# rosielab/emojivoice

Measured on AMD Instinct MI355X. Metric: audio_seconds_per_second, higher is better.
Workload: dtype f32 (deep layers: operand = two block-scaled fp16 pieces, product = 3 fp16 products on the fp16 MFMA, f32 accumulate); 1 GPU; config2: batch 64 x 516-frame (5.99 s) utterances per GPU, 10 Euler steps + HiFi-GAN V1, 22.05 kHz; global_batch=64, frames=516, ode_steps=10, parallelism=dp1, collective=none, batch_pipeline=cfm(i+1) || hifigan(i) on two streams, 2 pipeline(s) in flight

## Files before the change

emojivoice_amd/_lib.py:

```python
from __future__ import annotations

import ctypes as C
import os
import subprocess
from typing import Dict, Optional

import numpy as np
import torch

_HERE = os.path.dirname(os.path.abspath(__file__))
LIB_PATH = os.environ.get("EV_LIB_PATH") or os.path.join(_HERE, "lib", "libemojivoice_hip.so")
CSRC = os.path.join(_HERE, "csrc")
SOURCES = [os.path.join(CSRC, n) for n in ("ev_engine.hip", "ev_kernels.h", "ev_analysis_kernels.h", "ev_analysis.h")] \
    + [os.path.join(os.path.dirname(_HERE), "include", "emojivoice.h")]

EXPORTS = [
    "ev_abi_version", "ev_create", "ev_destroy", "ev_last_error", "ev_load_estimator", "ev_load_vocoder", "ev_load_vocoder_cfg", "ev_load_text_encoder", "ev_text_encoder",
    "ev_text_encoder_status", "ev_stft_magnitude", "ev_denoise", "ev_align", "ev_dbg_conv_bench",
    "ev_workspace_bytes", "ev_cfm_decode", "ev_estimator", "ev_hifigan", "ev_profile_enable", "ev_profile_read", "ev_profile_read_split", "ev_dbg_last_cfg", "ev_set_arithmetic", "ev_get_arithmetic",
    "ev_op_conv1d", "ev_op_groupnorm_mish", "ev_op_groupnorm_mish2", "ev_op_conv_groupnorm", "ev_op_layernorm", "ev_op_split_pieces", "ev_op_attention", "ev_op_ln_mlp", "ev_set_mrf_streams_max",
    "ev_cfm_decode2", "ev_reserve", "ev_alloc_count", "ev_dbg_sk_stats", "ev_op_attn_out", "ev_dbg_set_amax", "ev_dbg_set_attn_h16", "ev_dbg_set_chain", "ev_dbg_sk_taken",
    "ev_load_mel_basis", "ev_mel_spectrogram",
    "ev_maximum_path", "ev_log_prior", "ev_mas_align",
    "ev_estimator_rows", "ev_cfm_loss",
    "ev_load_resampler", "ev_resample", "ev_mel_stats",
    "ev_trim_bounds", "ev_trim_apply",
    "ev_pitch_yin", "ev_dtw",
    "ev_loudness",
    "ev_pyin_observe", "ev_pyin_decode",
    "ev_op_attention2", "ev_op_attn_out2",
    "ev_load_stoi", "ev_stoi",
    "ev_load_stft_dist", "ev_stft_dist",
    "ev_load_voice_quality", "ev_voice_quality",
    "ev_load_formants", "ev_formants",
    "ev_perturbation",
    "ev_load_harmonics", "ev_harmonics",
    "ev_functionals",
]


class EvLibraryError(RuntimeError):
    pass


class ev_tensor_index(C.Structure):
    _fields_ = [("name", C.c_char_p), ("offset", C.c_uint64), ("ndim", C.c_int32), ("shape", C.c_int64 * 4)]


class ev_model_dims(C.Structure):
    _fields_ = [("n_feats", C.c_int32), ("spk_emb_dim", C.c_int32), ("channels", C.c_int32), ("heads", C.c_int32),
                ("head_dim", C.c_int32)]


class ev_vocoder_config(C.Structure):
    _fields_ = [("resblock", C.c_int32), ("num_levels", C.c_int32), ("upsample_rates", C.c_int32 * 4), ("upsample_kernel_sizes", C.c_int32 * 4),
                ("resblock_kernel_sizes", C.c_int32 * 3), ("resblock_dilations", (C.c_int32 * 3) * 3)]


def vocoder_config(h) -> ev_vocoder_config:
    c = ev_vocoder_config()
# ... 94 lines not shown
    lib.ev_stoi.argtypes = [vp, vp, vp, vp, i32, i32, C.c_double, C.c_double, vp, vp, vp, vp, vp, vp]
    lib.ev_load_stft_dist.argtypes = [vp, vp, vp, i32, i32, i32]
    lib.ev_stft_dist.argtypes = [vp, vp, vp, vp, i32, i32, C.c_double, vp, vp, vp, vp]
    lib.ev_load_voice_quality.argtypes = [vp, vp, vp, i32, i32, i32, vp, vp, i32, i32, i32, vp, C.c_double]
    lib.ev_voice_quality.argtypes = [vp, vp, vp, i32, i32, C.c_double, vp, vp, vp, vp]
    lib.ev_load_formants.argtypes = [vp, vp, i32, i32, i32, C.c_double, C.c_double, C.c_double, i32]
    lib.ev_formants.argtypes = [vp, vp, vp, i32, i32, C.c_double, vp, vp, vp, vp]
    lib.ev_perturbation.argtypes = [vp, vp, vp, i32, i32, i32, vp, i32, i32, C.c_double, C.c_double, C.c_double, vp, vp, vp, vp]
    lib.ev_load_harmonics.argtypes = [vp, vp, vp, i32, i32, i32, C.c_double, i32, C.c_double, C.c_double, C.c_double]
    lib.ev_harmonics.argtypes = [vp, vp, vp, i32, i32, vp, vp, vp, i32, C.c_double, vp, vp, vp, vp]
    lib.ev_functionals.argtypes = [vp, vp, vp, vp, i32, i32, i32, vp, i32, vp, vp, vp]
    lib.ev_maximum_path.argtypes = [vp, vp, vp, vp, i32, i32, i32, vp, vp, vp]
    lib.ev_log_prior.argtypes = [vp, vp, vp, i32, i32, i32, vp, vp]
    lib.ev_mas_align.argtypes = [vp, vp, vp, vp, vp, i32, i32, i32, vp, vp, vp, vp, vp]
    lib.ev_profile_enable.argtypes = [vp, i32]
    lib.ev_profile_read.argtypes = [vp, C.POINTER(C.c_double), C.POINTER(C.c_double), C.POINTER(C.c_int64), i32]
    lib.ev_profile_read_split.argtypes = [vp, C.POINTER(C.c_double), C.POINTER(C.c_double), C.POINTER(C.c_int64)]
    lib.ev_dbg_last_cfg.argtypes = [vp]
    lib.ev_set_arithmetic.argtypes = [vp, i32]
    lib.ev_get_arithmetic.argtypes = [vp]
    lib.ev_dbg_set_amax.argtypes = [vp, i32]
    lib.ev_dbg_set_attn_h16.argtypes = [vp, i32]
    lib.ev_dbg_set_chain.argtypes = [vp, i32]
    lib.ev_dbg_sk_taken.argtypes = [vp]
    lib.ev_dbg_sk_taken.restype = C.c_int64
    lib.ev_op_conv1d.argtypes = [vp, vp, vp, vp, i32, i32, i32, i32, i32, i32, i32, i32, i32, f32, vp, vp]
    lib.ev_op_groupnorm_mish.argtypes = [vp, vp, vp, vp, vp, i32, i32, i32, i32, vp, vp]
    lib.ev_op_groupnorm_mish2.argtypes = [vp, vp, vp, vp, vp, i32, i32, i32, i32, i32, vp, i32, vp, vp, vp]
    lib.ev_op_conv_groupnorm.argtypes = [vp, vp, vp, vp, i32, i32, i32, vp, vp, vp, i32, vp, vp, vp, vp, vp, C.POINTER(C.c_int), vp]
    lib.ev_op_layernorm.argtypes = [vp, vp, vp, vp, i32, i32, vp, vp]
    lib.ev_op_split_pieces.argtypes = [vp, vp, i32, vp, vp]
    lib.ev_op_attention.argtypes = [vp, vp, vp, i32, i32, i32, vp, vp]
    lib.ev_op_attn_out.argtypes = [vp, vp, vp, i32, i32, vp, vp, vp, vp]
    lib.ev_op_attention2.argtypes = [vp, vp, vp, i32, i32, i32, i32, i32, i32, vp, C.POINTER(C.c_int), vp]
    lib.ev_op_attn_out2.argtypes = [vp, vp, vp, i32, i32, i32, i32, vp, vp, f32, f32, f32, vp, C.POINTER(C.c_int), vp]
    lib.ev_op_ln_mlp.argtypes = [vp, vp, vp, vp, vp, vp, vp, vp, vp, vp, vp, i32, i32, i32, vp, vp]
    for n in EXPORTS:
        getattr(lib, n)
    _lib = lib
    return lib


def _stream_ptr() -> int:
    return int(torch.cuda.current_stream().cuda_stream)


# ... 621 lines not shown
        return int(self.lib.ev_workspace_bytes(self.h, B, Tp, Tv))

    def profile_enable(self, on: bool):
        self._check(self.lib.ev_profile_enable(self.h, int(on)), "ev_profile_enable")

    def op_split_pieces(self, x):
        x = self._f32(x).reshape(-1)
        out = torch.empty((3, x.numel()), dtype=torch.float32, device=x.device)
        self._check(self.lib.ev_op_split_pieces(self.h, x.data_ptr(), x.numel(), out.data_ptr(), _stream_ptr()), "ev_op_split_pieces")
        return out

    def set_arithmetic(self, bf16_products: int):
        self._check(self.lib.ev_set_arithmetic(self.h, int(bf16_products)), "ev_set_arithmetic")

    def set_amax(self, on: bool) -> None:
        self._check(self.lib.ev_dbg_set_amax(self.h, int(bool(on))), "ev_dbg_set_amax")

    def set_attn_h16(self, on: bool) -> None:
        self._check(self.lib.ev_dbg_set_attn_h16(self.h, int(bool(on))), "ev_dbg_set_attn_h16")

    def set_chain(self, on: bool) -> None:
        self._check(self.lib.ev_dbg_set_chain(self.h, int(bool(on))), "ev_dbg_set_chain")

    def arithmetic(self) -> int:
        return int(self.lib.ev_get_arithmetic(self.h))

    def last_cfg(self) -> int:
        return int(self.lib.ev_dbg_last_cfg(self.h))

    def profile_read_split(self):
        ms, fl, n = C.c_double(), C.c_double(), C.c_int64()
        self._check(self.lib.ev_profile_read_split(self.h, C.byref(ms), C.byref(fl), C.byref(n)), "ev_profile_read_split")
        return ms.value, fl.value, n.value

    def profile_read(self, reset: bool = True):
        ms, fl, n = C.c_double(), C.c_double(), C.c_int64()
        self._check(self.lib.ev_profile_read(self.h, C.byref(ms), C.byref(fl), C.byref(n), int(reset)), "ev_profile_read")
        return ms.value, fl.value, n.value

    def op_conv1d(self, x, w, bias, dilation=1, transposed=False, stride=1, padding=0, pre_lrelu_slope=-1.0):
        x = self._f32(x)
        B, Cin, T = x.shape
        w = np.ascontiguousarray(w.detach().cpu().float().numpy())
        if transposed:
            Cout, K = w.shape[1], w.shape[2]
            Tout = T * stride
# ... 139 lines not shown
```

emojivoice_amd/csrc/ev_engine.hip:

```cpp
#include "ev_kernels.h"
#include "../../include/emojivoice.h"

#include <math.h>
#include <stdlib.h>
#include <stdarg.h>
#include <stdio.h>
#include <string.h>

#include <algorithm>
#include <atomic>
#include <mutex>
#include <numeric>
#include <string>
#include <unordered_map>
#include <vector>

namespace {

struct HostTensor {
    const float* p = nullptr;
    int ndim = 0;
    int64_t shape[4] = {0, 0, 0, 0};
    int64_t numel() const { int64_t n = 1; for (int i = 0; i < ndim; ++i) n *= shape[i]; return n; }
};
typedef std::unordered_map<std::string, HostTensor> TensorMap;

struct Geom { int nrows, S, P, T; };

struct ConvLayer {
    float* W = nullptr;
    unsigned short* Wh = nullptr; float wh_scale = 1.f;
    unsigned short* Wx = nullptr;
    unsigned short* Wq = nullptr;
    float* bias = nullptr;
    int2* taplist[3] = {nullptr, nullptr, nullptr};
    int* nact[3] = {nullptr, nullptr, nullptr};
    bool sparse_taps = false;
    bool tile128_exact = true;
    int kstack_mt = 0, kstack_tap = 0;
    int ntaps = 0, off[EV_MAX_TAPS] = {0};
    int halo_lo = 0, halo_hi = 0;
    bool wide = false;
    int Cin = 0, Cout = 0, Mpad = 0, Kpad = 0;
    double macs_per_row = 0;
};

struct Epi {
    int act = ACT_NONE; float act_slope = 0.f; const float* act_a = nullptr; const float* act_b = nullptr;
    int mask1 = 0; float scale = 1.f; const float* R = nullptr; int ldr = 0; int accum = 0; int div3 = 0;
    int act2_lrelu = 0; float act2_slope = 0.f; int mask2 = 0; const float* rowmask = nullptr; int mmul = 1;
    float* Y2 = nullptr; int ldy2 = 0;
    float pro_slope = -1.f;
    int dbg = 0; int force_cfg = -1; int stagger = -1; unsigned long long* stamps = nullptr;
    float* gn_part = nullptr;
    int isplit_log2 = 31, isstride = 0;
    unsigned* ymax = nullptr; int ymax_mul = 1; const unsigned* rmax = nullptr; const unsigned* yold = nullptr; const unsigned* xmax = nullptr; int xmax_n = 0;
    int osplit_log2 = 31, osstride = 0;
};

struct ResnetW { ConvLayer c1r, c2; float *g1, *b1, *g2, *b2; };
struct TransW {
    ConvLayer qkv, out, ff1, ff2; float *ln1g, *ln1b, *ln3g, *ln3b, *alpha, *binv;
    float qkv_scale[3] = {0.f, 0.f, 0.f};
};

struct EstimatorW {
    bool loaded = false;
    int in_ch = 0;
    ConvLayer t1, t2, tmlp;
    ResnetW rn[6];
    ConvLayer rn0_c1r_x, rn0_c1r_ms;
    TransW tr[6];
    ConvLayer down0, down1, up0, up1, fin_conv, fin_proj;
    float *fin_g, *fin_b;
};

struct VocoderW {
    bool loaded = false;
    int rb = 1;
    int nl = 4;
// ... 42 lines not shown
    StoiW stoi;
    StftDistW stftd;
    VoiceQW voiceq;
    FormantW fmt;
    HarmW harm;
    struct Scratch { char* p = nullptr; size_t bytes = 0; hipStream_t last = nullptr; bool last_valid = false; };
    Scratch dn_ws, enc_ws, mas_ws;
    Scratch dtw_ws;
    Scratch stat_ws;
    Scratch trim_ws;
    Scratch loud_ws;
    Scratch stoi_ws;
    Scratch stftd_ws;
    float* zeros = nullptr;
    int max_steps = 64;
    int* bad_ids_host = nullptr; int* bad_ids_dev = nullptr;
    char* ws = nullptr; size_t ws_bytes = 0; size_t ws_used = 0; size_t ws_bytes_last = 0;
    int ws_B = -1, ws_Tp = -1, ws_Tv = -1;
    bool prof = false;
    bool fuse_pairs = true;
    bool fuse_attn = true;
    bool attn_h16 = true;
    bool use_chain = true;
    bool fuse_mlp = true;
    int gn_stats_tiles = 0;
    int fuse_mlp_min_tiles = 96;
    std::vector<hipEvent_t> ev_pool; size_t ev_used = 0;
    hipStream_t ws_stream = nullptr; bool ws_stream_valid = false;
    float* temb_host[2] = {nullptr, nullptr}; size_t temb_cap[2] = {0, 0}; hipEvent_t temb_ev[2] = {nullptr, nullptr}; int temb_slot = 0;
    float* cap_pool = nullptr; size_t cap_stride = 0; int cap_used = 0; int cap_nt[8] = {0};
    struct TprojEntry { int nt; float* d; };
    std::vector<TprojEntry> tproj_cache;
    bool captured = false; int cap_B = 0, cap_Tp = 0;
    int64_t n_allocs = 0;
    double prof_flops = 0; int64_t prof_launches = 0;
    struct ProfRec { int kind, Cin, Cout, ntaps, nrows, cfg, lean; double flops; bool split = false; };
    std::vector<ProfRec> prof_recs;
    hipStream_t stream = nullptr;
    hipStream_t mrf_stream[2] = {nullptr, nullptr};
    hipEvent_t mrf_ev[4] = {nullptr, nullptr, nullptr, nullptr};
    int ncu = 0;
    unsigned* sk_ctrl = nullptr;
    unsigned sk_seq = 0;
    float* sk_part = nullptr;
    int split_terms = 16;
    bool use_amax = true;
// ... 247 lines not shown
            if ((r + p - k) % s == 0) {
                int o = (r + p - k) / s;
                bool found = false;
                for (int x : offs) if (x == o) found = true;
                if (!found) offs.push_back(o);
            }
    for (size_t i = 0; i < offs.size(); ++i) for (size_t j = i + 1; j < offs.size(); ++j) if (offs[j] < offs[i]) std::swap(offs[i], offs[j]);
    if ((int)offs.size() > EV_MAX_TAPS) return fail(h, "too many polyphase taps");
    L.Cin = Cin; L.Cout = s * Cout; L.ntaps = (int)offs.size(); L.Mpad = round_up(L.Cout, 128); L.Kpad = round_up(Cin, EV_BK);
    for (int i = 0; i < L.ntaps; ++i) L.off[i] = offs[i];
    std::vector<float> Wh((size_t)L.ntaps * L.Mpad * L.Kpad, 0.f), bh((size_t)L.Cout, 0.f);
    for (int r = 0; r < s; ++r)
        for (int k = 0; k < K; ++k) {
            if ((r + p - k) % s != 0) continue;
            const int o = (r + p - k) / s;
            int ti = 0;
            while (offs[ti] != o) ++ti;
            for (int co = 0; co < Cout; ++co)
                for (int ci = 0; ci < Cin; ++ci)
                    Wh[((size_t)ti * L.Mpad + r * Cout + co) * L.Kpad + ci] = w.p[((size_t)ci * Cout + co) * K + k];
        }
    if (b) for (int r = 0; r < s; ++r) for (int co = 0; co < Cout; ++co) bh[r * Cout + co] = b->p[co];
    L.macs_per_row = (double)Cin * Cout * K;
    return finish_layer(h, L, Wh, b ? &bh : nullptr);
}

int pack_conv_stride2(ev_handle* h, ConvLayer& L, const HostTensor& w, const HostTensor* b) {
    const int Cout = (int)w.shape[0], Cin = (int)w.shape[1], K = (int)w.shape[2];
    if (K != 3) return fail(h, "stride-2 conv expects k=3");
    L.Cin = 2 * Cin; L.Cout = Cout; L.ntaps = 2; L.off[0] = -1; L.off[1] = 0; L.Mpad = round_up(Cout, 128); L.Kpad = round_up(2 * Cin, EV_BK);
    std::vector<float> Wh((size_t)2 * L.Mpad * L.Kpad, 0.f), bh;
    for (int co = 0; co < Cout; ++co)
        for (int ci = 0; ci < Cin; ++ci) {
            const float* wk = &w.p[((size_t)co * Cin + ci) * 3];
            Wh[((size_t)0 * L.Mpad + co) * L.Kpad + Cin + ci] = wk[0];
            Wh[((size_t)1 * L.Mpad + co) * L.Kpad + ci] = wk[1];
            Wh[((size_t)1 * L.Mpad + co) * L.Kpad + Cin + ci] = wk[2];
        }
    if (b) bh.assign(b->p, b->p + Cout);
    L.macs_per_row = (double)Cout * Cin * 3;
    return finish_layer(h, L, Wh, b ? &bh : nullptr);
}

const HostTensor* find(ev_handle* h, const TensorMap& m, const std::string& k) {
    auto it = m.find(k);
    if (it == m.end()) { fail(h, "missing tensor '%s'", k.c_str()); return nullptr; }
// ... 80 lines not shown
    dispatch<1, 2, 3, 0, EPI_FULL>(epi_flavour(p, lo.lean && lean_ok(p)), [&](auto E) {
        launch<conv_gemm_kernel<BM, BN, WM, WN, PF, E == EPI_FULL, (E > 0 ? E : 0)>>(lo.device, dim3(p.mtiles * p.ntiles), dim3(256), smem, st, p);
    });
}

template <int BM, int BN, int WM, int WN, int TERMS = 6>
void launch_split(const ConvParams& p, hipStream_t st, const LaunchOpts& lo) {
    const size_t xs = (size_t)(BN + ((lo.halo + 7) & ~7)) * EVX_RSB;
    constexpr size_t es = (size_t)4 * 32 * (BM / WM + 4) * sizeof(float);
    const size_t smem = xs > es ? xs : es;
    dispatch<1, 2, 3>(epi_flavour(p, true), [&](auto E) {
        launch<conv_split_kernel<BM, BN, WM, WN, E, TERMS>>(lo.device, dim3(p.mtiles * p.ntiles), dim3(256), smem, st, p);
    });
}
template <int BM, int BN, int WM, int WN>
void launch_h16(const ConvParams& p, hipStream_t st, const LaunchOpts& lo) {
    const size_t xs = (size_t)(BN + EV_HALO) * EVH_RSB + 16;
    constexpr size_t es = (size_t)4 * 32 * (BM / WM + 4) * sizeof(float);
    const size_t smem = xs > es ? xs : es;
    const dim3 grid(p.mtiles * p.ntiles);
    if (p.Wq && p.act != ACT_SNAKE)
        dispatch<1, 3>(epi_flavour(p, true), [&](auto E) { launch<conv_h16_kernel<BM, BN, WM, WN, E, 1>>(lo.device, grid, dim3(256), smem, st, p); });
    else dispatch<1, 2, 3>(epi_flavour(p, true), [&](auto E) { launch<conv_h16_kernel<BM, BN, WM, WN, E>>(lo.device, grid, dim3(256), smem, st, p); });
}
inline bool split_ok(const ConvLayer& L, const ConvParams& p0) {
    ConvParams p = p0;
    p.dbg &= ~4;
    return L.Wx && lean_ok(p) && (p.isplit_log2 >= 31 || (p.isplit_log2 >= 6 && p.isplit_log2 < 31)) && L.Cin % EVX_KC == 0 && L.Cin == L.Kpad && L.Mpad % 128 == 0 && ((size_t)p.bias & 15) == 0;
}

template <int TW>
void launch_sk(const ConvParams& p, hipStream_t st, const LaunchOpts& lo) {
    constexpr int KS = TW == 4 ? 4 : 8, BN = TW == 4 ? 64 : 32;
    const int nchunks = p.Kpad / EV_BK, rows = BN + ((lo.halo + 7) & ~7);
    int kbs = nchunks < (TW == 4 ? 8 : 32) ? nchunks : (TW == 4 ? 8 : 32);
    while (kbs > 8 && ((size_t)rows * (32 * kbs + 4) * 4 > 150 * 1024 || rows * kbs * 8 > EV_SK_MAXF4(TW))) kbs = (kbs - 1) & ~7;
    const size_t xs = 2 * EV_MAX_TAPS + (size_t)rows * (32 * kbs + 4);
    const size_t red = (size_t)(KS - 1) * TW * 16 * 64, es = (size_t)TW * 32 * 36;
    size_t smem = std::max(xs, std::max(red, es)) * sizeof(float);
    ConvParams q = p;
    q.sk_kb = kbs;
    dispatch<1, 2, 3, 0, EPI_FULL>(epi_flavour(p, lo.lean && lean_ok(p)), [&](auto E) {
        launch<conv_gemm_sk_kernel<KS, E == EPI_FULL, (E > 0 ? E : 0), TW>>(lo.device, dim3(p.mtiles * p.ntiles), dim3(64 * TW * KS), smem, st, q);
    });
}

// ... 38 lines not shown
    else if (BN + p.halo_lo + p.halo_hi <= 16 * 9)
        dispatch<1, 3>(lean, [&](auto E) { launch<conv_h16_bal_kernel<BM, BN, WM, WN, E, 9>>(lo.device, grid, block, smem, h->stream, p); });
    else dispatch<1, 3>(lean, [&](auto E) { launch<conv_h16_bal_kernel<BM, BN, WM, WN, E>>(lo.device, grid, block, smem, h->stream, p); });
    return 0;
}
inline bool split_bal_ok(const ev_handle* h, const ConvLayer& L, const ConvParams& p, long nwg, int wpc) {
    return h->sk_balance && h->ncu > 0 && split_ok(L, p) && p.act != ACT_SNAKE && !p.dbg && !p.stamps && !p.gn_part &&
           nwg * 2 >= h->ncu && wpc * h->ncu <= EV_SK_MAXWG && (long)nwg * (p.Kpad / EVX_KC) >= (long)wpc * h->ncu;
}
inline bool bal_ok(const ev_handle* h, const ConvLayer& L, const ConvParams& p, long nwg, int wpc) {
    if (L.sparse_taps) return false;
    return h->sk_balance && h->ncu > 0 && lean_ok(p) && p.act != ACT_SNAKE && !p.dbg && !p.stamps && !p.gn_part &&
           nwg >= h->ncu && nwg < 4L * wpc * h->ncu && wpc * h->ncu <= EV_SK_MAXWG && (long)nwg * (p.Kpad / EV_BK) >= (long)wpc * h->ncu;
}

enum : int {
    CFG_128x128 = 0, CFG_64x128 = 1, CFG_32x256 = 2, CFG_64x192 = 5, CFG_64x64 = 6,
    CFG_64x64_PF = 8,
    CFG_SK64 = 9, CFG_SK32 = 19,
    CFG_SPLIT = 40, CFG_SPLIT64 = 41, CFG_SPLIT3 = 43, CFG_SPLIT9 = 49,
    CFG_H16 = 46,
    CFG_SPLIT_BAL = 60,
    CFG_H16_64 = 47, CFG_BAL64 = 56, CFG_H16_BAL = 66,
};
struct ConvTile { int cfg, bm, bn, slots; bool split; };
constexpr ConvTile EV_TILES[] = {
    {CFG_128x128, 128, 128, 3, false}, {CFG_64x128, 64, 128, 4, false}, {CFG_32x256, 32, 256, 3, false}, {CFG_64x192, 64, 192, 4, false},
    {CFG_64x64, 64, 64, 5, false}, {CFG_64x64_PF, 64, 64, 5, false}, {CFG_SK64, 64, 64, 0, false}, {CFG_SK32, 32, 32, 0, false},
    {CFG_SPLIT, 128, 128, 0, true}, {CFG_SPLIT64, 64, 128, 0, true}, {CFG_SPLIT3, 128, 128, 0, true}, {CFG_H16, 128, 128, 0, true},
    {CFG_SPLIT9, 128, 128, 0, true}, {CFG_SPLIT_BAL, 128, 128, 0, true},
};
inline const ConvTile* conv_tile(int cfg) {
    for (const ConvTile& t : EV_TILES) if (t.cfg == cfg) return &t;
    return nullptr;
}
inline int tile_list(const ConvTile& t) { return t.bm == 128 ? 0 : t.bm == 64 ? 1 : 2; }
inline int tile_mtiles(const ConvTile& t, const ConvLayer& L) { return t.bm == 128 ? L.Mpad / 128 : (L.Cout + t.bm - 1) / t.bm; }
inline long tile_count(const ConvTile& t, const ConvLayer& L, const Geom& g) { return (long)tile_mtiles(t, L) * ((g.nrows + t.bn - 1) / t.bn); }

int pick_cfg(const ev_handle* h, const ConvLayer& L, const ConvParams& p, const Geom& g) {
    auto tiles = [&](int cfg) { return tile_count(*conv_tile(cfg), L, g); };
    int cfg;
    if (L.Cout <= 32) cfg = CFG_32x256;
    else {
        double best = 1e30;
        cfg = CFG_64x128;
// ... 9 lines not shown
        }
    }
    if (L.sparse_taps && L.Cout > 32 && tiles(CFG_64x64) <= 256L * 5 * 2) cfg = CFG_64x64;
    if (cfg == CFG_64x64 && tiles(CFG_64x64) <= 320) cfg = CFG_64x64_PF;
    if (cfg == CFG_64x128 && L.Cout % 128 == 0 && !L.sparse_taps && tiles(CFG_64x128) >= 256L * 4 * 6)
        cfg = (L.Cin > 128 && L.ntaps >= 7) ? CFG_64x192 : CFG_128x128;
    if (h->small_sk) {
        const long wg64 = tiles(CFG_64x64);
        if ((cfg == CFG_64x64 || cfg == CFG_64x64_PF) && wg64 <= 192 && (L.Kpad / EV_BK) * L.ntaps >= 8) cfg = CFG_SK64;
        if ((cfg == CFG_64x64 || cfg == CFG_64x64_PF) && wg64 <= 96 && L.Kpad == 128 && L.Cin == 128 && !L.sparse_taps) cfg = CFG_SK64;
        if (cfg == CFG_SK64 && wg64 <= 192 && L.Cout >= 32) cfg = CFG_SK32;
    }
    {
        const int split_terms = h->split_terms;
        const bool fp32_tile = cfg == CFG_128x128 || cfg == CFG_64x128 || cfg == CFG_64x192 || cfg == CFG_64x64;
        const long nwg128 = tiles(CFG_128x128);
        if (split_terms > 0 && fp32_tile && split_ok(L, p) && L.Cout % 128 == 0 && (!L.sparse_taps || (L.tile128_exact && L.kstack_mt == 0)) && nwg128 >= 2L * 2 * h->ncu && h->ncu > 0)
            cfg = split_terms == 3 ? CFG_SPLIT3 : split_terms == 9 ? CFG_SPLIT9 : split_terms == 16 ? CFG_H16 : CFG_SPLIT;
        else if ((split_terms == 6 || split_terms == 3 || split_terms == 16) && fp32_tile && split_ok(L, p) && L.Cout % 64 == 0 && L.kstack_mt == 0 && h->ncu > 0 &&
                 (L.sparse_taps || L.Cout % 128 != 0) && tiles(CFG_64x128) >= 2L * 3 * h->ncu) cfg = CFG_SPLIT64;
        else if ((split_terms == 6 || split_terms == 16) && fp32_tile && L.Cout == L.Mpad && split_bal_ok(h, L, p, nwg128, 2)) cfg = CFG_SPLIT_BAL;
    }
    return cfg;
}

constexpr int EV_GN_MAXTILES = 256;
int launch_conv(ev_handle* h, const ConvLayer& L, const float* X, int ldx, float* Y, int ldy, const Geom& g, const Epi& e) {
    ConvParams p;
    memset(&p, 0, sizeof p);
    h->gn_stats_tiles = 0;
    if (L.halo_lo + L.halo_hi > EV_HALO) return fail(h, "launch_conv: conv halo %d exceeds EV_HALO", L.halo_lo + L.halo_hi);
    p.X = X; p.ldx = ldx; p.Cin = L.Cin; p.isplit_log2 = e.isplit_log2; p.isstride = e.isstride;
    p.W = L.W; p.Wx = L.Wx; p.Wh = L.Wh; p.Wq = L.Wq; p.wh_scale = L.wh_scale; p.Mpad = L.Mpad; p.Kpad = L.Kpad; p.bias = L.bias;
    p.Y = Y; p.ldy = ldy; p.Cout = L.Cout; p.osplit_log2 = e.osplit_log2; p.osstride = e.osstride; p.mmul = e.mmul;
    p.nrows = g.nrows; p.S = g.S; p.P = g.P; p.T = g.T;
    p.ntaps = L.ntaps; for (int i = 0; i < L.ntaps; ++i) p.off[i] = L.off[i];
    if (!L.sparse_taps || L.kstack_mt > 0) {
        bool even = true;
        const int d = L.ntaps > 1 ? L.off[1] - L.off[0] : 0;
        for (int i = 2; i < L.ntaps; ++i) even = even && (L.off[i] - L.off[i - 1] == d);
        if (even) {
            p.plane_bytes = (L.Mpad / 32) * (L.Kpad / 8) * 1024; p.koff0 = L.off[0]; p.kdoff = d;
            if (!L.sparse_taps) p.ktaps_n = L.ntaps;
            else { p.kstack_mt = L.kstack_mt; p.kstack_tap = L.kstack_tap; }
        }
    }
// ... 4 lines not shown
    p.act2_lrelu = e.act2_lrelu; p.act2_slope = e.act2_slope; p.mask2 = e.mask2; p.rowmask = e.rowmask;
    p.Y2 = e.Y2; p.ldy2 = e.ldy2; p.dbg = e.dbg; p.stamps = e.stamps;
    p.xmax = e.xmax; p.xmax_n = e.xmax_n; p.rmax = e.rmax; p.yold = e.yold; p.ymax_mul = e.ymax_mul; h->amax_emitted = false;
    if ((ldx & 3) || (L.Cin & 3)) return fail(h, "conv input must be float4-aligned (ldx %d Cin %d)", ldx, L.Cin);
    if (over_4gib(g, ldx) || over_4gib(g, ldy) || (e.R && over_4gib(g, e.ldr)) || (e.Y2 && over_4gib(g, e.ldy2)))
        return fail(h, "tensor of %.1f GiB exceeds the 4 GiB buffer-addressing limit: split the batch", (double)g.nrows * std::max(ldx, ldy) * 4.0 / 1073741824.0);

    int cfg = pick_cfg(h, L, p, g);
    LaunchOpts lo;
    lo.device = h->device; lo.lean = h->lean; lo.halo = L.halo_lo + L.halo_hi;
    if (h->force_cfg >= 0) cfg = h->force_cfg;
    if (e.force_cfg >= 0) { cfg = e.force_cfg < 1000 ? e.force_cfg % 100 : -1; lo.wgs_per_cu = (e.force_cfg / 100) % 10; }
    if ((h->force_cfg >= 0 || e.force_cfg >= 0) && !conv_tile(cfg))
        return fail(h, "launch_conv: forced tile configuration %d is not one launch_conv selects", e.force_cfg >= 0 ? e.force_cfg : h->force_cfg);
    if (prof_begin(h)) return 1;
    {
        const ConvTile& s = *conv_tile(cfg == CFG_SK64 ? CFG_32x256 : cfg);
        p.stagger_slots = tile_count(s, L, g) >= 256L * s.slots * 3 ? s.slots : 0;
        if (e.stagger >= 0) p.stagger_slots = e.stagger;
    }
    if (conv_tile(cfg)->split && !split_ok(L, p)) cfg = CFG_128x128;
    if (cfg == CFG_H16 && !L.Wh) cfg = CFG_SPLIT;
    const bool fp16 = h->split_terms == 16 && L.Wh;
    {
        const bool lean1or3 = lean_ok(p) && p.act != ACT_SNAKE && h->lean;
        const bool h16 = cfg == CFG_H16 || (cfg == CFG_SPLIT64 && fp16);
        const bool gemm = (cfg == CFG_128x128 || cfg == CFG_64x128 || cfg == CFG_64x192 || cfg == CFG_64x64) && lean1or3;
        const bool no_amax = !h->use_amax;
        if (!no_amax && e.ymax && lean1or3 && (h16 || gemm) && (!e.R || e.rmax) && (!e.accum || e.yold)) { p.ymax = e.ymax; h->amax_emitted = true; }
        if (no_amax) p.xmax = nullptr;
    }
    const ConvTile& t = *conv_tile(cfg);
    p.mtiles = tile_mtiles(t, L); p.ntiles = (g.nrows + t.bn - 1) / t.bn;
    p.taplist = L.taplist[tile_list(t)]; p.nact_tab = L.nact[tile_list(t)]; p.tl_stride = L.sparse_taps ? EV_MAX_TAPS : 0;
    switch (cfg) {
    case CFG_H16: launch_h16<128, 128, 2, 2>(p, h->stream, lo); break;
    case CFG_SPLIT64:
        if (fp16) { launch_h16<64, 128, 2, 2>(p, h->stream, lo); cfg = CFG_H16_64; }
        else if (h->split_terms == 3) launch_split<64, 128, 2, 2, 3>(p, h->stream, lo);
        else launch_split<64, 128, 2, 2, 6>(p, h->stream, lo);
        break;
    case CFG_SPLIT_BAL:
        if (fp16) { if (launch_bal<PIPE_H16, 128, 128, 2, 2>(h, p, lo, 2)) return 1; cfg = CFG_H16_BAL; }
        else if (launch_bal<PIPE_BF16, 128, 128, 2, 2>(h, p, lo, 2)) return 1;
        break;
    case CFG_SPLIT: launch_split<128, 128, 2, 2, 6>(p, h->stream, lo); break;
    case CFG_SPLIT3: launch_split<128, 128, 2, 2, 3>(p, h->stream, lo); break;
    case CFG_SPLIT9: launch_split<128, 128, 2, 2, 9>(p, h->stream, lo); break;
    case CFG_128x128: launch_cfg<128, 128, 2, 2>(p, h->stream, lo); break;
    case CFG_64x128: launch_cfg<64, 128, 2, 2>(p, h->stream, lo); break;
    case CFG_64x192: launch_cfg<64, 192, 2, 2>(p, h->stream, lo); break;
    case CFG_64x64_PF: launch_cfg<64, 64, 2, 2, true>(p, h->stream, lo); break;
    case CFG_SK64: launch_sk<4>(p, h->stream, lo); break;
// ... 942 lines not shown
    return 0;
}

}

extern "C" {

int ev_abi_version(void) { return EV_ABI_VERSION; }

int ev_create(ev_handle** out, int device, const ev_model_dims* dims) {
    if (!out || !dims) return 1;
    *out = nullptr;
    int ndev = 0;
    if (hipGetDeviceCount(&ndev) != hipSuccess || device < 0 || device >= ndev) return 2;
    if (hipSetDevice(device) != hipSuccess) return 3;
    ev_handle* h = new ev_handle();
    h->device = device;
    h->dims = *dims;
    { const char* fp = getenv("EV_FUSE_PAIRS"); if (fp && *fp == '0') h->fuse_pairs = false; }
    { const char* fp = getenv("EV_FUSE_MLP"); if (fp && *fp == '0') h->fuse_mlp = false; }
    { const char* fp = getenv("EV_FUSE_ATTN"); if (fp && *fp == '0') h->fuse_attn = false; }
    if (getenv("EV_NO_ATTN_H16")) h->attn_h16 = false;
    if (getenv("EV_NO_CHAIN")) h->use_chain = false;
    { const char* fp = getenv("EV_FUSE_MLP_MIN"); if (fp && *fp) h->fuse_mlp_min_tiles = atoi(fp); }
    { const char* fp = getenv("EV_MRF_STREAMS_MAX"); if (fp && *fp) h->mrf_max_frames = atoi(fp); }
    if (getenv("EV_NO_AMAX")) h->use_amax = false;
    { const char* sp = getenv("EV_SPLIT"); if (sp && *sp) { const int t = atoi(sp); h->split_terms = (t == 0 || t == 3 || t == 6 || t == 9 || t == 16) ? t : 16; } }
    { const char* fp = getenv("EV_NO_SK_BALANCE"); if (fp && *fp && *fp != '0') h->sk_balance = false; }
    { const char* fp = getenv("EV_SK_SPIN"); if (fp && *fp) h->sk_spin = atoi(fp); }
    { const char* fp = getenv("EV_SK_WGS"); if (fp && *fp) h->sk_wgs = std::min(3, std::max(1, atoi(fp))); }
    { const char* fp = getenv("EV_FORCE_CFG"); if (fp && *fp) h->force_cfg = atoi(fp); }
    if (getenv("EV_NO_LEAN")) h->lean = false;
    if (getenv("EV_NO_SK")) h->small_sk = false;
    if (getenv("EV_NO_SK32_LEAN")) h->sk32_lean = false;
    if (getenv("EV_NO_GN_STATS")) h->gn_stats = false;
    if (getenv("EV_NO_QKV_H16")) h->qkv_h16 = false;
    if (getenv("EV_NO_ATTN_SK")) h->attn_sk = false;
    { const char* fp = getenv("EV_ATTN_TPW"); if (fp) h->attn_tpw = std::max(1, atoi(fp)); }
    if (getenv("EV_FULL_REZERO")) h->full_rezero = true;
    { const char* fp = getenv("EV_RB2_MINKEEP"); if (fp) h->rb2_minkeep = atoi(fp); }
    if (hipDeviceGetAttribute(&h->ncu, hipDeviceAttributeMultiprocessorCount, device) != hipSuccess) h->ncu = 0;
    if (dims->n_feats != 80 || dims->channels != 256 || dims->head_dim != 64 || dims->heads != 2) {
        delete h;
        return 4;
    }
    *out = h;
// ... 768 lines not shown
    int cin = w.ch[0];
    const bool ms = mrf_streams_for(h, B, T) && !h->prof && v.Pax[0][1] != nullptr;
    if (ms && !h->mrf_stream[0]) {
        for (int c = 0; c < 2; ++c) HIPCHK(h, hipStreamCreateWithFlags(&h->mrf_stream[c], hipStreamNonBlocking));
        for (int c = 0; c < 4; ++c) HIPCHK(h, hipEventCreateWithFlags(&h->mrf_ev[c], hipEventDisableTiming));
    }
    if (ms) HIPCHK(h, hipStreamSynchronize(h->stream));
    hipStream_t s0 = h->stream;
    struct StreamGuard {
        ev_handle* h; hipStream_t s; bool bal; bool ms; bool done;
        ~StreamGuard() {
            h->stream = s; h->sk_balance = bal;
            if (ms && !done) { for (int c = 0; c < 2; ++c) if (h->mrf_stream[c]) (void)hipStreamSynchronize(h->mrf_stream[c]); }
        }
    } guard{h, s0, h->sk_balance, ms, false};
    if (ms) h->sk_balance = false;
    const int nl = w.nl;
    for (int i = 0; i < nl; ++i) {
        const int l = i + 1, C = w.ch[l], s = w.ups[i].Cout / C;
        const float next_slope = (l == nl) ? 0.01f : 0.1f;
        {
            Epi e;
            with_slots(e, xin, nullptr, v.U[l], s);
            if (launch_conv(h, w.ups[i], xin, cin, v.U[l], s * C, v.g[l - 1], e)) return 1;
            wrote(v.U[l], false);
        }
        if (ms) {
            HIPCHK(h, hipEventRecord(h->mrf_ev[3], s0));
            for (int c = 0; c < 2; ++c) HIPCHK(h, hipStreamWaitEvent(h->mrf_stream[c], h->mrf_ev[3], 0));
        }
        for (int j = 0; j < 3; ++j) {
            const float* x = v.U[l];
            const bool own = ms && j > 0;
            h->stream = own ? h->mrf_stream[j - 1] : s0;
            float* pp[2] = {own ? v.Pax[j - 1][l] : v.Pa[l], own ? v.Pbx[j - 1][l] : v.Pb[l]};
            float* t1 = own ? v.T1x[j - 1][l] : v.T1[l];
            if (w.rb == 2) {
                const int b = i * 3 + j;
                auto join = [&](Epi& e) {
                    e.accum = (j > 0);
                    if (j == 2) { e.div3 = 1; e.act2_lrelu = 1; e.act2_slope = next_slope; }
                };
                if (rb2_ok(h, w.c1[b], C)) {
                    if (ms && j > 0) HIPCHK(h, hipStreamWaitEvent(h->stream, h->mrf_ev[j - 1], 0));
                    Epi e; join(e);
                    float* y = v.XS[l];
// ... 138 lines not shown
int ev_dbg_last_cfg(ev_handle* h) { return h ? h->last_cfg : -1; }

int ev_set_arithmetic(ev_handle* h, int bf16_products) {
    if (!h) return 1;
    if (bf16_products != 0 && bf16_products != 3 && bf16_products != 6 && bf16_products != 9 && bf16_products != 16)
        return fail(h, "ev_set_arithmetic: 0, 3, 6, 9 or 16, got %d", bf16_products);
    h->split_terms = bf16_products;
    return 0;
}
int ev_get_arithmetic(ev_handle* h) { return h ? h->split_terms : -1; }

int ev_dbg_set_amax(ev_handle* h, int on) {
    if (!h) return 1;
    h->use_amax = on != 0;
    return 0;
}

int ev_dbg_set_chain(ev_handle* h, int on) {
    if (!h) return 1;
    h->use_chain = on != 0;
    return 0;
}

int ev_dbg_set_attn_h16(ev_handle* h, int on) {
    if (!h) return 1;
    h->attn_h16 = on != 0;
    return 0;
}

int ev_profile_read_split(ev_handle* h, double* ms_out, double* flops_out, int64_t* launches_out) {
    if (!h) return 1;
    HIPCHK(h, hipStreamSynchronize(h->stream));
    double ms = 0, fl = 0;
    int64_t n = 0;
    if (h->prof_recs.size() * 2 == h->ev_used)
        for (size_t i = 0; i < h->prof_recs.size(); ++i) {
            const auto& r = h->prof_recs[i];
            if (!r.split) continue;
            float t = 0;
            HIPCHK(h, hipEventElapsedTime(&t, h->ev_pool[2 * i], h->ev_pool[2 * i + 1]));
            ms += t; fl += r.flops; n += 1;
        }
    if (ms_out) *ms_out = ms;
    if (flops_out) *flops_out = fl;
    if (launches_out) *launches_out = n;
    return 0;
// ... 394 lines not shown
```

emojivoice_amd/csrc/ev_kernels.h:

```cpp
#pragma once
#include <hip/hip_runtime.h>
#include <stdint.h>
#include <type_traits>

typedef float f32x16 __attribute__((ext_vector_type(16)));
typedef float f32x4 __attribute__((ext_vector_type(4)));
typedef int i32x4 __attribute__((ext_vector_type(4)));

#define EV_MAX_TAPS 16
#define EV_BK 32
#define EV_LDK 36
#define EV_WROWS 128
#define EV_SK_MAXF4(TW) ((TW) == 4 ? (64 + 64) * 8 * 8 : 16 * 512)
#define EV_HALO 64

enum { ACT_NONE = 0, ACT_LRELU = 1, ACT_TANH = 2, ACT_SILU = 3, ACT_MISH = 4, ACT_SNAKE = 5 };

struct SkCtl {
    unsigned* ctrl;
    unsigned* flags;
    float* part;
    int part_floats;
    int q, r;
    int spin_limit;
// ... 1418 lines not shown
                const unsigned nap = have_next ? q_off(ntv.x, last_tap ? ch * 2 + 2 : ch * 2) : q_off(tv_first.x, 0);
                ldQB(QB1, brow, 1);
                __builtin_amdgcn_sched_barrier(0);
                mmaQ(QA0, QB0);
                __builtin_amdgcn_sched_barrier(0);
                ldQA(QA0, nap);
                ldQB(QB0, nbrow, 0);
                __builtin_amdgcn_sched_barrier(0);
                mmaQ(QA1, QB1);
                __builtin_amdgcn_sched_barrier(0);
                ldQA(QA1, nap + 2048u);
                brow = nbrow;
            }
        }
#pragma unroll
        for (int a = 0; a < QM; ++a)
#pragma unroll
            for (int b = 0; b < QN; ++b) acc[a][b] *= acc_out;
        __builtin_amdgcn_s_setprio(3);
        ev_amax_from_acc_q<QM, QN>(p, am, acc, c.row0(n0), lane);
        conv_epilogue_lean_q<TM, TN, LEAN>(p, acc, c.epi(smem), c.ch0(m0), c.row0(n0), lane);
        ev_amax_emit(p, am, c.row0(n0), TN * 32, lane);
    }
}

template <int BM, int BN, int WAVES_M, int WAVES_N, int LEAN, int TERMS = 6>
__global__ __launch_bounds__(256, 2) void conv_split_bal_kernel(const ConvParams p) {
    constexpr int TM = BM / WAVES_M / 32;
    constexpr int TN = BN / WAVES_N / 32;
    static_assert(WAVES_M * WAVES_N == 4 && TM >= 1 && TN >= 1 && LEAN != 0, "balanced build: 4 waves, lean epilogue");
    extern __shared__ __attribute__((aligned(16))) float smem[];
    char* Xb = (char*)smem;
    const int tid = threadIdx.x;
    const int lane = tid & 63;
    const int wave = __builtin_amdgcn_readfirstlane(tid >> 6);
    const int wm = wave / WAVES_N, wn = wave % WAVES_N;
    const int li = lane & 31, lh = lane >> 5;
    const int nchunks = p.Kpad / EVX_KC;
    const int g = blockIdx.x;
    const unsigned tag = sk_tag(p.sk);
    int u = sk_start(p.sk, g);
    const int ue = sk_start(p.sk, g + 1);
    const __amdgpu_buffer_rsrc_t rPart = ev_rsrc(p.sk.part), rW = ev_rsrc(p.Wx), rX = ev_rsrc(p.X);
    const unsigned pslot = (unsigned)p.sk.part_floats * 8u;
    constexpr int PN = TM * TN * 4;
    const unsigned pelem = (unsigned)(wave * PN) * 1024u + (unsigned)lane * 16u;
// ... 4141 lines not shown
```

include/emojivoice.h:

```cpp
#ifndef EMOJIVOICE_H
#define EMOJIVOICE_H

#include <stddef.h>
#include <stdint.h>

#ifdef __cplusplus
extern "C" {
#endif

#define EV_ABI_VERSION 4

typedef struct ev_handle ev_handle;

typedef struct ev_tensor_index {
    const char *name;
    uint64_t offset;
    int32_t ndim;
    int64_t shape[4];
} ev_tensor_index;

typedef struct ev_model_dims {
    int32_t n_feats;
    int32_t spk_emb_dim;
    int32_t channels;
// ... 139 lines not shown
                 const float *d_period ,
                 const double *d_formant , const int32_t *d_fcount , int n_formants,
                 double power_floor, double *d_frame , int32_t *d_count ,
                 double *d_harm , void *stream);

int ev_functionals(ev_handle *h, const double *d_v , const uint8_t *d_mask ,
                   const int32_t *d_len , int B, int K, int F,
                   const double *q , int NQ,
                   double *d_stat , int32_t *d_count , void *stream);

int ev_profile_enable(ev_handle *h, int on);
int ev_profile_read(ev_handle *h, double *conv_ms, double *conv_flops, int64_t *conv_launches, int reset);
int ev_profile_read_split(ev_handle *h, double *ms, double *flops, int64_t *launches);
int ev_set_arithmetic(ev_handle *h, int setting);
int ev_get_arithmetic(ev_handle *h);

int ev_dbg_last_cfg(ev_handle *h);

int ev_dbg_conv_bench(ev_handle *h, int Cin, int Cout, int K, int dil, int B, int T, int P, int iters, int dbg, int cfg, float *ms_out);

int ev_dbg_set_amax(ev_handle *h, int on);
int ev_dbg_set_attn_h16(ev_handle *h, int on);
int ev_dbg_set_chain(ev_handle *h, int on);

int ev_dbg_sk_stats(ev_handle *h, uint32_t *out3);
int64_t ev_dbg_sk_taken(ev_handle *h);

int ev_op_conv1d(ev_handle *h, const float *d_x , const float *w ,
                 const float *bias , int B, int Cin, int T, int Cout, int K, int dilation,
                 int transposed, int stride, int padding, float pre_lrelu_slope , float *d_y, void *stream);
int ev_op_groupnorm_mish(ev_handle *h, const float *d_x , const float *d_gamma, const float *d_beta,
                         const int32_t *d_lengths, int B, int C, int T, int groups, float *d_y, void *stream);
int ev_op_groupnorm_mish2(ev_handle *h, const float *d_x , const float *d_gamma, const float *d_beta,
                          const int32_t *d_lengths, int B, int C, int T, int groups, int mode, const float *d_temb,
                          int temb_stride, const float *d_R, float *d_y, void *stream);
int ev_op_conv_groupnorm(ev_handle *h, const float *d_x , const float *w ,
                         const float *bias , int Cin, int T, int K, const float *d_gamma,
                         const float *d_beta, const int32_t *d_lengths , int mode, const float *d_temb, const float *d_R,
                         float *d_conv, float *d_part, float *d_y, int *tiles_out, void *stream);
int ev_op_split_pieces(ev_handle *h, const float *d_x, int n, float *d_pieces, void *stream);
int ev_op_layernorm(ev_handle *h, const float *d_x , const float *d_gamma, const float *d_beta, int rows,
                    int C, float *d_y, void *stream);
int ev_op_ln_mlp(ev_handle *h, const float *d_x, const float *d_ln_g, const float *d_ln_b, const float *w1, const float *b1,
                 const float *d_alpha_exp, const float *d_beta_inv, const float *w2, const float *b2, const float *d_rowmask,
                 int rows, int M1, int mode, float *d_y, void *stream);
int ev_op_attention(ev_handle *h, const float *d_qkv , const int32_t *d_lengths, int B, int T,
// ... 15 lines not shown
```

Baseline: 4744 audio_s/s.

## Add specialized fp16 transposed-conv kernel for stride-2 HiFi-GAN upsample layers

```diff
diff --git a/emojivoice_amd/_lib.py b/emojivoice_amd/_lib.py
--- a/emojivoice_amd/_lib.py
+++ b/emojivoice_amd/_lib.py
@@ -36,6 +36,7 @@
     "ev_perturbation",
     "ev_load_harmonics", "ev_harmonics",
     "ev_functionals",
+    "ev_dbg_set_convt", "ev_dbg_convt_launches",
 ]
 
 
@@ -176,6 +177,9 @@
     lib.ev_dbg_set_amax.argtypes = [vp, i32]
     lib.ev_dbg_set_attn_h16.argtypes = [vp, i32]
     lib.ev_dbg_set_chain.argtypes = [vp, i32]
+    lib.ev_dbg_set_convt.argtypes = [vp, i32]
+    lib.ev_dbg_convt_launches.argtypes = [vp]
+    lib.ev_dbg_convt_launches.restype = C.c_int64
     lib.ev_dbg_sk_taken.argtypes = [vp]
     lib.ev_dbg_sk_taken.restype = C.c_int64
     lib.ev_op_conv1d.argtypes = [vp, vp, vp, vp, i32, i32, i32, i32, i32, i32, i32, i32, i32, f32, vp, vp]
@@ -843,6 +847,12 @@
     def set_chain(self, on: bool) -> None:
         self._check(self.lib.ev_dbg_set_chain(self.h, int(bool(on))), "ev_dbg_set_chain")
 
+    def set_convt(self, mode: int) -> None:
+        self._check(self.lib.ev_dbg_set_convt(self.h, int(mode)), "ev_dbg_set_convt")
+
+    def convt_launches(self) -> int:
+        return int(self.lib.ev_dbg_convt_launches(self.h))
+
     def arithmetic(self) -> int:
         return int(self.lib.ev_get_arithmetic(self.h))
 
diff --git a/emojivoice_amd/csrc/ev_engine.hip b/emojivoice_amd/csrc/ev_engine.hip
--- a/emojivoice_amd/csrc/ev_engine.hip
+++ b/emojivoice_amd/csrc/ev_engine.hip
@@ -43,6 +43,7 @@
     bool wide = false;
     int Cin = 0, Cout = 0, Mpad = 0, Kpad = 0;
     double macs_per_row = 0;
+    int convt_s = 0, convt_k = 0;
 };
 
 struct Epi {
@@ -56,6 +57,7 @@
     int isplit_log2 = 31, isstride = 0;
     unsigned* ymax = nullptr; int ymax_mul = 1; const unsigned* rmax = nullptr; const unsigned* yold = nullptr; const unsigned* xmax = nullptr; int xmax_n = 0;
     int osplit_log2 = 31, osstride = 0;
+    bool convt_auto = false;
 };
 
 struct ResnetW { ConvLayer c1r, c2; float *g1, *b1, *g2, *b2; };
@@ -144,6 +146,9 @@
     bool fuse_attn = true;
     bool attn_h16 = true;
     bool use_chain = true;
+    int convt_mode = 1;
+    int convt_bn = 0;
+    int64_t convt_launches = 0;
     bool fuse_mlp = true;
     int gn_stats_tiles = 0;
     int fuse_mlp_min_tiles = 96;
@@ -437,6 +442,7 @@
         }
     if (b) for (int r = 0; r < s; ++r) for (int co = 0; co < Cout; ++co) bh[r * Cout + co] = b->p[co];
     L.macs_per_row = (double)Cin * Cout * K;
+    L.convt_s = s; L.convt_k = K;
     return finish_layer(h, L, Wh, b ? &bh : nullptr);
 }
 
@@ -563,6 +569,12 @@
     if (p.Wq && p.act != ACT_SNAKE)
         dispatch<1, 3>(epi_flavour(p, true), [&](auto E) { launch<conv_h16_kernel<BM, BN, WM, WN, E, 1>>(lo.device, grid, dim3(256), smem, st, p); });
     else dispatch<1, 2, 3>(epi_flavour(p, true), [&](auto E) { launch<conv_h16_kernel<BM, BN, WM, WN, E>>(lo.device, grid, dim3(256), smem, st, p); });
+}
+template <int CIN, int BN>
+void launch_convt2(const ConvParams& p, hipStream_t st, const LaunchOpts& lo) {
+    constexpr int WPC = CIN == 128 ? (BN == 128 ? 2 : 4) : 4;
+    constexpr size_t xs = (size_t)(BN + 2) * (4 * CIN + 16) + 32, es = (size_t)4 * 32 * (CIN / 2 + 4) * sizeof(float);
+    launch<convt2_h16_kernel<CIN, BN, WPC>>(lo.device, dim3((p.nrows + BN - 1) / BN), dim3(256), xs > es ? xs : es, st, p);
 }
 inline bool split_ok(const ConvLayer& L, const ConvParams& p0) {
     ConvParams p = p0;
@@ -647,6 +659,7 @@
     CFG_H16 = 46,
     CFG_SPLIT_BAL = 60,
     CFG_H16_64 = 47, CFG_BAL64 = 56, CFG_H16_BAL = 66,
+    CFG_CONVT2 = 48,
 };
 struct ConvTile { int cfg, bm, bn, slots; bool split; };
 constexpr ConvTile EV_TILES[] = {
@@ -702,6 +715,18 @@
         else if ((split_terms == 6 || split_terms == 16) && fp32_tile && L.Cout == L.Mpad && split_bal_ok(h, L, p, nwg128, 2)) cfg = CFG_SPLIT_BAL;
     }
     return cfg;
+}
+
+inline int convt2_bn(const ev_handle* h, const ConvLayer& L, const ConvParams& p, const Epi& e, int cfg) {
+    if (h->convt_mode == 0 || h->force_cfg >= 0 || e.force_cfg >= 0 || h->split_terms != 16 || !L.Wh || !h->lean) return 0;
+    if (L.convt_s != 2 || L.convt_k != 4 || L.ntaps != 3 || L.off[0] != -1 || L.off[1] != 0 || L.off[2] != 1) return 0;
+    if ((L.Cin != 64 && L.Cin != 128) || L.Cin != L.Kpad || L.Cout != L.Cin || L.Mpad != 128 || !L.sparse_taps || L.kstack_mt != 0) return 0;
+    const int list = L.Cin == 128 ? 1 : 2;
+    if (!L.taplist[list] || !L.nact[list] || !L.bias) return 0;
+    if (!split_ok(L, p) || p.isplit_log2 < 31 || p.osplit_log2 < 31 || p.ldx < L.Cin || p.ldy < L.Cout) return 0;
+    if (p.act != ACT_NONE || p.R || lean_acc(p) || p.mask1 || p.mask2 || p.dbg || p.stamps || p.gn_part || p.P < 1) return 0;
+    if (h->convt_mode == 1 && (!e.convt_auto || cfg != CFG_SPLIT64)) return 0;
+    return h->convt_bn ? h->convt_bn : 128;
 }
 
 constexpr int EV_GN_MAXTILES = 256;
@@ -752,13 +777,25 @@
     if (conv_tile(cfg)->split && !split_ok(L, p)) cfg = CFG_128x128;
     if (cfg == CFG_H16 && !L.Wh) cfg = CFG_SPLIT;
     const bool fp16 = h->split_terms == 16 && L.Wh;
+    const int ct_bn = convt2_bn(h, L, p, e, cfg);
     {
         const bool lean1or3 = lean_ok(p) && p.act != ACT_SNAKE && h->lean;
-        const bool h16 = cfg == CFG_H16 || (cfg == CFG_SPLIT64 && fp16);
+        const bool h16 = cfg == CFG_H16 || (cfg == CFG_SPLIT64 && fp16) || ct_bn > 0;
         const bool gemm = (cfg == CFG_128x128 || cfg == CFG_64x128 || cfg == CFG_64x192 || cfg == CFG_64x64) && lean1or3;
         const bool no_amax = !h->use_amax;
         if (!no_amax && e.ymax && lean1or3 && (h16 || gemm) && (!e.R || e.rmax) && (!e.accum || e.yold)) { p.ymax = e.ymax; h->amax_emitted = true; }
         if (no_amax) p.xmax = nullptr;
+    }
+    if (ct_bn > 0) {
+        const int list = L.Cin == 128 ? 1 : 2;
+        p.mtiles = 1; p.ntiles = (g.nrows + ct_bn - 1) / ct_bn;
+        p.taplist = L.taplist[list]; p.nact_tab = L.nact[list]; p.tl_stride = EV_MAX_TAPS;
+        if (L.Cin == 128) { if (ct_bn == 128) launch_convt2<128, 128>(p, h->stream, lo); else launch_convt2<128, 64>(p, h->stream, lo); }
+        else { if (ct_bn == 128) launch_convt2<64, 128>(p, h->stream, lo); else launch_convt2<64, 64>(p, h->stream, lo); }
+        HIPCHK(h, hipGetLastError());
+        ++h->convt_launches;
+        h->last_cfg = CFG_CONVT2;
+        return h->prof ? prof_end(h, {0, L.Cin, L.Cout, L.ntaps, g.nrows, CFG_CONVT2, 1, 2.0 * L.macs_per_row * valid_rows(g), true}) : 0;
     }
     const ConvTile& t = *conv_tile(cfg);
     p.mtiles = tile_mtiles(t, L); p.ntiles = (g.nrows + t.bn - 1) / t.bn;
@@ -1747,6 +1784,8 @@
     { const char* fp = getenv("EV_FUSE_ATTN"); if (fp && *fp == '0') h->fuse_attn = false; }
     if (getenv("EV_NO_ATTN_H16")) h->attn_h16 = false;
     if (getenv("EV_NO_CHAIN")) h->use_chain = false;
+    if (getenv("EV_NO_CONVT")) h->convt_mode = 0;
+    if (const char* bn = getenv("EV_CONVT_BN")) { const int v = atoi(bn); if (v == 64 || v == 128) h->convt_bn = v; }
     { const char* fp = getenv("EV_FUSE_MLP_MIN"); if (fp && *fp) h->fuse_mlp_min_tiles = atoi(fp); }
     { const char* fp = getenv("EV_MRF_STREAMS_MAX"); if (fp && *fp) h->mrf_max_frames = atoi(fp); }
     if (getenv("EV_NO_AMAX")) h->use_amax = false;
@@ -2561,6 +2600,7 @@
         {
             Epi e;
             with_slots(e, xin, nullptr, v.U[l], s);
+            e.convt_auto = true;
             if (launch_conv(h, w.ups[i], xin, cin, v.U[l], s * C, v.g[l - 1], e)) return 1;
             wrote(v.U[l], false);
         }
@@ -2745,6 +2785,13 @@
     return 0;
 }
 
+int ev_dbg_set_convt(ev_handle* h, int mode) {
+    if (!h || mode < 0 || mode > 2) return 1;
+    h->convt_mode = mode;
+    return 0;
+}
+int64_t ev_dbg_convt_launches(ev_handle* h) { return h ? h->convt_launches : -1; }
+
 int ev_dbg_set_attn_h16(ev_handle* h, int on) {
     if (!h) return 1;
     h->attn_h16 = on != 0;
diff --git a/emojivoice_amd/csrc/ev_kernels.h b/emojivoice_amd/csrc/ev_kernels.h
--- a/emojivoice_amd/csrc/ev_kernels.h
+++ b/emojivoice_amd/csrc/ev_kernels.h
@@ -1464,6 +1464,126 @@
         conv_epilogue_lean_q<TM, TN, LEAN>(p, acc, c.epi(smem), c.ch0(m0), c.row0(n0), lane);
         ev_amax_emit(p, am, c.row0(n0), TN * 32, lane);
     }
+}
+
+template <int CIN>
+struct EvPipeH16W {
+    static constexpr int PIECES = 2, KC = CIN, RSB = 4 * CIN + 16;
+    static constexpr unsigned KG_BYTES = 2048u;
+    static __device__ __forceinline__ unsigned tap_off(unsigned tb) { return tb; }
+    template <int TM, int TN>
+    static __device__ __forceinline__ void mma(f32x16 (&acc)[TM][TN], const f32x4 (&a)[2][TM], const f32x4 (&b)[2][TN]) { evh_mma<TM, TN>(acc, a, b); }
+    static __device__ __forceinline__ void put(char* Xb, int r, int sc4, bool on, const f32x4 v ) {
+        uint2 q0v, q1v;
+        evh_split4(v, q0v, q1v);
+        if (on) {
+            char* dst = Xb + r * RSB + sc4 * 2;
+            *(uint2*)(dst) = q0v; *(uint2*)(dst + KC * 2) = q1v;
+        }
+    }
+};
+template <int CIN, int BN, int WPC>
+__global__ __launch_bounds__(256, WPC) void convt2_h16_kernel(const ConvParams p) {
+    using Pipe = EvPipeH16W<CIN>;
+    using Core = EvConvCore<CIN, BN, 2, 2, Pipe>;
+    constexpr int TM = Core::TM, TN = Core::TN, RPS = Core::RPS, RSB = Pipe::RSB;
+    constexpr int XROWS = BN + 2, NP = (XROWS + RPS - 1) / RPS, NCH = CIN / EVX_KC;
+    static_assert((CIN == 64 || CIN == 128) && (BN == 64 || BN == 128), "convt2_h16_kernel shapes");
+    extern __shared__ __attribute__((aligned(16))) float smem[];
+    char* Xb = (char*)smem;
+    float* red = smem + (XROWS * RSB) / 4;
+
+    const int n0 = blockIdx.x * BN;
+    if (ev_tile_is_padding(p.S, p.P, p.T, p.nrows, n0, BN)) return;
+    Core c(p, 0);
+    const int lane = c.lane, wave = c.wave, srow = c.srow, sc4 = c.sc4;
+    EvAmax am = ev_amax_begin(p, c.row0(n0), TN * 32);
+    const int2* tl = p.taplist + (size_t)c.wm * p.tl_stride;
+    const int nact = __builtin_amdgcn_readfirstlane(p.nact_tab[c.wm]);
+    const __amdgpu_buffer_rsrc_t rW = ev_rsrc(p.Wh), rX = ev_rsrc(p.X);
+    const int2 tlv = (lane < nact) ? tl[lane] : make_int2(0, 0);
+    const int2 tv_first = ev_tap_at(tlv, 0);
+    if (nact > 0) c.ring_fill(rW, tv_first.x);
+
+    unsigned xoff[NP];
+    ev_row_offs<RPS>(p, n0 - 1 + srow, XROWS, sc4, xoff);
+    f32x4 xg[NP];
+#pragma unroll
+    for (int q = 0; q < NP; ++q) xg[q] = ev_bload4(rX, xoff[q], 0);
+    if ((NP - 1) * RPS + srow >= XROWS) { const f32x4 z = {0.f, 0.f, 0.f, 0.f}; xg[NP - 1] = z; }
+    float mx = p.xmax ? ev_amax_read(p, n0 - 1, n0 + BN, lane) : -1.f;
+    if (mx < 0.f) {
+        float m = 0.f;
+#pragma unroll
+        for (int q = 0; q < NP; ++q) m = fmaxf(m, evh_absmax4(xg[q]));
+        mx = evh_wg_max(red, 0, wave, lane, m);
+    }
+    if (!evh_is_finite(mx)) {
+        float m = 0.f;
+#pragma unroll
+        for (int q = 0; q < NP; ++q) m = fmaxf(m, evh_absmax4_finite(xg[q]));
+        mx = evh_wg_max(red, 4, wave, lane, m);
+    }
+    const float xs = evh_scale_for(mx);
+    const float acc_in = p.wh_scale * xs;
+    const float acc_out = 1.0f / acc_in;
+    __builtin_amdgcn_s_setprio(3);
+#pragma unroll
+    for (int q = 0; q < NP; ++q) {
+        const int r = q * RPS + srow;
+        Pipe::put(Xb, r, sc4, r < XROWS, ev_pro_lrelu4(p, xg[q]) * xs);
+    }
+    ev_lds_barrier();
+    __builtin_amdgcn_s_setprio(0);
+
+    c.acc_init(p, 0, acc_in, true);
+    const char* bbase = c.bbase(Xb, 1);
+    for (int ch = 0; ch < NCH; ++ch) {
+        const char* bb = bbase + ch * (EVX_KC * 2);
+        const char* brow = c.tap_first(tv_first, bb);
+        for (int ti = 0; ti < nact; ++ti) brow = c.tap(rW, tlv, tv_first, nact, ti, ch, NCH, bb, brow);
+    }
+#pragma unroll
+    for (int a = 0; a < TM; ++a)
+#pragma unroll
+        for (int b = 0; b < TN; ++b)
+#pragma unroll
+            for (int r = 0; r < 16; ++r) c.acc[a][b][r] *= acc_out;
+    __builtin_amdgcn_s_setprio(3);
+    ev_amax_from_acc<TM, TN>(p, am, c.acc, c.row0(n0), lane);
+    {
+        constexpr int EC = TM * 32, ELD = EC + 4, C4 = EC / 4, RPP = 64 / C4, NPS = 32 / RPP;
+        float* Es = c.epi(smem);
+        const int li = lane & 31, lh = lane >> 5, er = lane / C4, ec = (lane % C4) * 4;
+        const int nw0 = c.row0(n0);
+        const __amdgpu_buffer_rsrc_t rY = ev_rsrc(p.Y);
+        int t = (nw0 + er) % p.S - p.P;
+        const int lim = p.S - p.P;
+        unsigned yoff = ((unsigned)(nw0 + er) * (unsigned)p.ldy + (unsigned)(c.ch0(0) + ec)) * 4u;
+        const unsigned ystep = (unsigned)(RPP * p.ldy) * 4u;
+        ev_lds_barrier();
+#pragma unroll
+        for (int j = 0; j < TN; ++j) {
+#pragma unroll
+            for (int i = 0; i < TM; ++i)
+#pragma unroll
+                for (int g = 0; g < 4; ++g) {
+                    const f32x4 q4 = {c.acc[i][j][4 * g], c.acc[i][j][4 * g + 1], c.acc[i][j][4 * g + 2], c.acc[i][j][4 * g + 3]};
+                    *(f32x4*)(Es + li * ELD + i * 32 + 8 * g + 4 * lh) = q4;
+                }
+            asm volatile("s_waitcnt lgkmcnt(0)" ::: "memory");
+#pragma unroll
+            for (int q = 0; q < NPS; ++q) {
+                const int n = nw0 + er + (j * NPS + q) * RPP;
+                const f32x4 v = *(const f32x4*)(Es + (q * RPP + er) * ELD + ec);
+                if (t >= 0 && t < p.T && n < p.nrows) ev_bstore4(rY, yoff, v);
+                t += RPP; t -= (t >= lim) ? p.S : 0; t -= (t >= lim) ? p.S : 0;
+                yoff += ystep;
+            }
+            asm volatile("s_waitcnt lgkmcnt(0)" ::: "memory");
+        }
+    }
+    ev_amax_emit(p, am, c.row0(n0), TN * 32, lane);
 }
 
 template <int BM, int BN, int WAVES_M, int WAVES_N, int LEAN, int TERMS = 6>
diff --git a/include/emojivoice.h b/include/emojivoice.h
--- a/include/emojivoice.h
+++ b/include/emojivoice.h
@@ -185,6 +185,8 @@
 int ev_dbg_set_amax(ev_handle *h, int on);
 int ev_dbg_set_attn_h16(ev_handle *h, int on);
 int ev_dbg_set_chain(ev_handle *h, int on);
+int ev_dbg_set_convt(ev_handle *h, int mode);
+int64_t ev_dbg_convt_launches(ev_handle *h);
 
 int ev_dbg_sk_stats(ev_handle *h, uint32_t *out3);
 int64_t ev_dbg_sk_taken(ev_handle *h);
```

Measured after the change: 4762 audio_s/s, median of 6. Within noise of the previous version (+0.4%).
